# SebastianHafner/multimodal_siamese_cd

Hardware: AMD Instinct MI355X
Metric: image-pairs/sec training step, 256×256 SAR+optical Siamese U-Net, 1/2/4/8 MI355X (higher is better)
Workload: dtype f32 (h2 split-fp16); 1 GPU; baseline_siamese: siameseunet TOPOLOGY [64, 128, 256, 512], 5-ch SAR+optical, 256x256, bs=32/GPU, conv math h2, fp32 activation storage, train step incl. AdamW; global_batch=32, tile=256, parallelism=dp1

## Files before the change

### multimodal_siamese_cd_amd/csrc/bn_f32.hip

```cpp
#include "common.h"

namespace scd {

constexpr int BN_THREADS = 256;
constexpr int BN_CHUNK_MAX = 4096;
constexpr int BN_CHUNK_MIN = 64;
constexpr int BN_TARGET_BLOCKS = 2048;

struct BnGeom {
    int64_t pseg;
    int chunk;
    int ncps;
    int nrec;
    int qpb;
    int cgroups;
};

static BnGeom bn_geom(const scd_nhwc_t &y, int nseg) {
    BnGeom g;
    g.pseg = pixels(y) / nseg;
    const int cq = y.c / 4;
    int q = 1;
    while (q * 2 <= cq && q * 2 <= 64) q *= 2;
    g.qpb = q;
    g.cgroups = (cq + q - 1) / q;
    int chunk = BN_CHUNK_MAX;
    while (chunk > BN_CHUNK_MIN && int64_t(nseg) * ((g.pseg + chunk - 1) / chunk) * g.cgroups < BN_TARGET_BLOCKS)
        chunk /= 2;
    g.chunk = chunk;
    g.ncps = int((g.pseg + chunk - 1) / chunk);
    g.nrec = nseg * g.ncps;
    return g;
}

typedef float f4 __attribute__((ext_vector_type(4)));

__device__ __forceinline__ f4 fabs4(f4 v) { return f4{fabsf(v.x), fabsf(v.y), fabsf(v.z), fabsf(v.w)}; }
__device__ __forceinline__ f4 fmax4(f4 a, f4 b) {
    return f4{fmaxf(a.x, b.x), fmaxf(a.y, b.y), fmaxf(a.z, b.z), fmaxf(a.w, b.w)};
}
#define PIN4(a, b, c, d) asm volatile("" : "+v"(a), "+v"(b), "+v"(c), "+v"(d))

struct Welford4 {
    float n;
    f4 mean, m2;
};

__device__ __forceinline__ void chan_merge(Welford4 &a, const Welford4 &b) {
    if (b.n == 0.f) return;
    if (a.n == 0.f) {
        a = b;
        return;
// ... 80 lines not shown
        __syncthreads();
    }
    if (pl == 0 && c < C) {
        const Welford4 a = sh[tid];
        const float mv[4] = {a.mean.x, a.mean.y, a.mean.z, a.mean.w};
        const float qv[4] = {a.m2.x, a.m2.y, a.m2.z, a.m2.w};
#pragma unroll
        for (int k = 0; k < 4; ++k) {
            float *r = rec + (size_t(c + k) * nrec + blockIdx.x) * 3;
            r[0] = a.n;
            r[1] = mv[k];
            r[2] = qv[k];
        }
    }
}

struct DWelford {
    double n, mean, m2;
};
__device__ __forceinline__ void dmerge(DWelford &a, const DWelford &b) {
    if (b.n == 0) return;
    if (a.n == 0) {
        a = b;
        return;
    }
    const double n = a.n + b.n;
    const double d = b.mean - a.mean;
    a.mean += d * b.n / n;
    a.m2 += b.m2 + d * d * a.n * b.n / n;
    a.n = n;
}

__device__ __forceinline__ DWelford block_dmerge(DWelford w, DWelford *sh) {
#pragma unroll
    for (int off = 1; off < 64; off <<= 1) {
        const DWelford o{__shfl_xor(w.n, off), __shfl_xor(w.mean, off), __shfl_xor(w.m2, off)};
        dmerge(w, o);
    }
    const int t = threadIdx.x;
    if ((t & 63) == 0) sh[t >> 6] = w;
    __syncthreads();
    DWelford a = sh[0];
    if (t == 0)
        for (int k = 1; k < BN_THREADS / 64; ++k) dmerge(a, sh[k]);
    __syncthreads();
    return a;
}

__device__ __forceinline__ float bn_act_bound(double n, double gamma, double beta, double shift) {
    const double dev = fabs(gamma) * sqrt(n > 1 ? n - 1 : 0.0);
    return float((dev + fabs(beta)) * (1.0 + 0x1p-10) + (fabs(shift) + fabs(beta)) * 0x1p-16);
}

__global__ __launch_bounds__(BN_THREADS) void bn_stats_finalize(const float *__restrict__ rec, int C, int nseg,
                                                                int ncps, int nrec, const float *gamma,
                                                                const float *beta, float eps, float momentum,
                                                                int update, float *rmean, float *rvar, float *smean,
                                                                float *sinv, float *scale, float *shift,
                                                                float *act_bound) {
    __shared__ DWelford sh[BN_THREADS / 64];
    const int c = blockIdx.x;
    const int t = threadIdx.x;
    const float *rc = rec + size_t(c) * nrec * 3;
    for (int s = 0; s < nseg; ++s) {
        DWelford w{0, 0, 0};
        for (int k = t; k < ncps; k += BN_THREADS) {
            const float *r = rc + size_t(s * ncps + k) * 3;
            dmerge(w, DWelford{r[0], r[1], r[2]});
        }
        const DWelford a = block_dmerge(w, sh);
        if (t == 0) {
            const double g = gamma ? gamma[c] : 1.0, b = beta ? beta[c] : 0.0;
            const double var = a.n > 0 ? a.m2 / a.n : 0.0;
            const double inv = 1.0 / sqrt(var + double(eps));
            smean[s * C + c] = float(a.mean);
            sinv[s * C + c] = float(inv);
            const float sc = float(g * inv);
            scale[s * C + c] = sc;
            shift[s * C + c] = float(b - a.mean * double(sc));
            if (act_bound) atomic_max_bound(act_bound, bn_act_bound(a.n, g, b, double(shift[s * C + c])));
            if (update) {
                const double uvar = a.n > 1 ? a.m2 / (a.n - 1) : var;
                rmean[c] = float((1.0 - momentum) * rmean[c] + momentum * a.mean);
                rvar[c] = float((1.0 - momentum) * rvar[c] + momentum * uvar);
            }
        }
    }
}

__global__ __launch_bounds__(BN_THREADS) void bn_tile_merge(const float *__restrict__ trec, int C, int tiles_per_seg,
                                                            int group, int ncps, int nrec, float tile_px,
                                                            float *__restrict__ rec) {
    const int c = blockIdx.y * BN_THREADS + threadIdx.x;
    if (c >= C) return;
    const int g = blockIdx.x;
    const int seg = g / ncps, k = g - (g / ncps) * ncps;
    const int t0 = seg * tiles_per_seg + k * group;
    const int t1 = min(t0 + group, (seg + 1) * tiles_per_seg);
    float n = 0.f, mean = 0.f, m2 = 0.f;
    auto merge = [&](float2 r) {
        const float nn = n + tile_px;
        const float d = r.x - mean;
        mean += d * (tile_px / nn);
        m2 += r.y + d * d * (n * tile_px / nn);
        n = nn;
    };
    int t = t0;
    for (; t + 8 <= t1; t += 8) {
        float2 r[8];
#pragma unroll
        for (int u = 0; u < 8; ++u) r[u] = *reinterpret_cast<const float2 *>(trec + (size_t(t + u) * C + c) * 2);
#pragma unroll
        for (int u = 0; u < 8; ++u) merge(r[u]);
    }
    for (; t < t1; ++t) merge(*reinterpret_cast<const float2 *>(trec + (size_t(t) * C + c) * 2));
    float *o = rec + (size_t(c) * nrec + g) * 3;
    o[0] = n;
    o[1] = mean;
    o[2] = m2;
}

__global__ void bn_eval_coeffs_kernel(int C, const float *gamma, const float *beta, const float *rm, const float *rv,
                                      float eps, float *scale, float *shift) {
    const int c = blockIdx.x * blockDim.x + threadIdx.x;
    if (c >= C) return;
    const double inv = 1.0 / sqrt(double(rv[c]) + double(eps));
    const float sc = float((gamma ? gamma[c] : 1.0f) * inv);
    scale[c] = sc;
    shift[c] = float((beta ? beta[c] : 0.0f) - double(rm[c]) * sc);
}

__device__ __forceinline__ float bn_relu(float y, float sc, float sh) { return fmaxf(fmaf(y, sc, sh), 0.f); }
__device__ __forceinline__ f4 bn_relu4(f4 y, f4 sc, f4 sh) {
    return f4{bn_relu(y.x, sc.x, sh.x), bn_relu(y.y, sc.y, sh.y), bn_relu(y.z, sc.z, sh.z), bn_relu(y.w, sc.w, sh.w)};
}

template <class T>
__global__ __launch_bounds__(256) void bn_relu_apply_kernel(const T *__restrict__ y, int ldy, T *__restrict__ a,
                                                            int lda, int C, int64_t pseg, const float *__restrict__ scale,
                                                            const float *__restrict__ shift) {
    const int seg = blockIdx.y;
    const int cq = C / 4;
    const int64_t total = pseg * cq;
    const float *sc = scale + seg * C;
    const float *sh = shift + seg * C;
    for (int64_t e = blockIdx.x * int64_t(blockDim.x) + threadIdx.x; e < total; e += int64_t(gridDim.x) * blockDim.x) {
        const int64_t p = seg * pseg + e / cq;
        const int c = int(e % cq) * 4;
        st4(a + p * lda + c, bn_relu4(ld4(y + p * ldy + c), ld4(sc + c), ld4(sh + c)));
    }
}


template <class T>
struct DaPlain {
    const T *da;
    int ldda;
    __device__ __forceinline__ void bind(int) {}
    __device__ __forceinline__ f4 operator()(int64_t p, int c) const { return ld4(da + p * ldda + c); }
};
template <class T>
struct DaPooled {
    const T *gy;
    const uint8_t *idx;
    int hy, wy, ldgy;
    const T *gs;
    int gsn, ldgs, skip_mode;
    const T *gs2;
    int ldgs2;
    int hx, wx, C;
    FastDiv div_hw, div_w, div_gsn;
    __device__ __forceinline__ void bind(int) {}
// ... 566 lines not shown
#pragma unroll
            for (int k = 0; k < NO; ++k) hw[k] += (a0 * k0[k] + a1 * k1[k]) + (a2 * k2[k] + a3 * k3[k]);
        }
        for (; p < ch.end; p += npl) {
            const f4 y0 = ld4(y + p * ldy + c);
            f4 k0[NO];
            const f4 z0 = relu_mask(y0, sc, sf, px(p, y0, k0));
            s1 += z0;
            s2 += z0 * ((y0 - mu) * iv);
            const f4 a0 = bn_relu4(y0, sc, sf);
#pragma unroll
            for (int k = 0; k < NO; ++k) hw[k] += a0 * k0[k];
        }
    }
    sh1[tid] = s1;
    sh2[tid] = s2;
#pragma unroll
    for (int k = 0; k < NO; ++k) shh[k][tid] = hw[k];
    __syncthreads();
    for (int off = npl / 2; off > 0; off >>= 1) {
        if (pl < off) {
            sh1[tid] += sh1[tid + off * qpb];
            sh2[tid] += sh2[tid + off * qpb];
#pragma unroll
            for (int k = 0; k < NO; ++k) shh[k][tid] += shh[k][tid + off * qpb];
        }
        __syncthreads();
    }
    if (pl == 0 && c < C) {
        const f4 a = sh1[tid], b = sh2[tid];
        const float av[4] = {a.x, a.y, a.z, a.w}, bv[4] = {b.x, b.y, b.z, b.w};
#pragma unroll
        for (int k = 0; k < 4; ++k) {
            float *r = rec + (size_t(c + k) * nrec + blockIdx.x) * 2;
            r[0] = av[k];
            r[1] = bv[k];
        }
#pragma unroll
        for (int o = 0; o < NO; ++o) {
            const f4 h = shh[o][tid];
            const float hv[4] = {h.x, h.y, h.z, h.w};
#pragma unroll
            for (int k = 0; k < 4; ++k) hrec[(size_t(o) * C + c + k) * nrec + blockIdx.x] = hv[k];
        }
    }
}

__device__ __forceinline__ float bn_dy_bound(double da_bound, double n, double gamma, double mean, double inv, double k1,
                                             double k2) {
    const double xhat = sqrt(n > 1 ? n - 1 : 0.0) * (1.0 + 0x1p-10) + fabs(mean) * inv * 0x1p-20 + 1.0;
    return float(fabs(gamma * inv) * (da_bound + fabs(k1) + xhat * fabs(k2)) * (1.0 + 0x1p-10));
}

__global__ __launch_bounds__(BN_THREADS) void bn_bwd_finalize(const float *__restrict__ rec, int C, int nseg,
                                                              int ncps, int nrec, int64_t pseg, float *coef,
                                                              float *dgamma, float *dbeta, const float *gamma = nullptr,
                                                              const float *sinv = nullptr, float *dbias = nullptr,
                                                              const float *smean = nullptr,
                                                              const float *da_bound = nullptr,
                                                              float *dy_bound = nullptr) {
    __shared__ double a1[BN_THREADS], a2[BN_THREADS];
    const int c = blockIdx.x;
    const int t = threadIdx.x;
    const float *rc = rec + size_t(c) * nrec * 2;
    double tg = 0, tb = 0, db = 0;
    for (int s = 0; s < nseg; ++s) {
        double s1[4] = {0, 0, 0, 0}, s2[4] = {0, 0, 0, 0};
        const float2 *rs = reinterpret_cast<const float2 *>(rc) + size_t(s) * ncps;
        int k = t;
        for (; k + 3 * BN_THREADS < ncps; k += 4 * BN_THREADS) {
            float2 v[4];
#pragma unroll
            for (int u = 0; u < 4; ++u) v[u] = rs[k + u * BN_THREADS];
#pragma unroll
            for (int u = 0; u < 4; ++u) {
                s1[u] += v[u].x;
                s2[u] += v[u].y;
            }
        }
        for (int u = 0; k < ncps; k += BN_THREADS, ++u) {
            const float2 v = rs[k];
            s1[u] += v.x;
            s2[u] += v.y;
        }
        double v1 = (s1[0] + s1[1]) + (s1[2] + s1[3]), v2 = (s2[0] + s2[1]) + (s2[2] + s2[3]);
#pragma unroll
        for (int off = 1; off < 64; off <<= 1) {
            v1 += __shfl_xor(v1, off);
            v2 += __shfl_xor(v2, off);
        }
        if ((t & 63) == 0) {
            a1[t >> 6] = v1;
            a2[t >> 6] = v2;
        }
        __syncthreads();
        if (t == 0) {
            for (int k = 1; k < BN_THREADS / 64; ++k) {
                a1[0] += a1[k];
                a2[0] += a2[k];
            }
            const float k1 = float(a1[0] / double(pseg));
            const float k2 = float(a2[0] / double(pseg));
            coef[(s * C + c) * 2 + 0] = k1;
            coef[(s * C + c) * 2 + 1] = k2;
            if (dy_bound) atomic_max_bound(dy_bound, bn_dy_bound(double(*da_bound), double(pseg), gamma ? gamma[c] : 1.0,
                                                                 smean[s * C + c], sinv[s * C + c], k1, k2));
            tb += a1[0];
            tg += a2[0];
            if (dbias) {
                const float mul = (gamma ? gamma[c] : 1.f) * sinv[s * C + c];
                db += double(mul) * (a1[0] - double(pseg) * double(k1));
            }
        }
        __syncthreads();
    }
    if (t == 0) {
        if (dgamma) dgamma[c] = float(tg);
        if (dbeta) dbeta[c] = float(tb);
        if (dbias) dbias[c] = float(db);
    }
}

template <class T, class DA>
__global__ __launch_bounds__(BN_THREADS) void bn_bwd_apply(const T *__restrict__ y, int ldy, DA da,
                                                           T *__restrict__ dy, int lddy, int C, int64_t pseg,
                                                           int ncps, int chunk, int nrec, int qpb, const float *smean,
                                                           const float *sinv, const float *gamma, const float *scale,
                                                           const float *shift, const float *coef,
                                                           float *__restrict__ brec, float *dy_bound) {
    __shared__ f4 sh[BN_THREADS];
    const int tid = threadIdx.x;
    const int q = tid % qpb, pl = tid / qpb, npl = BN_THREADS / qpb;
    const int c = (blockIdx.y * qpb + q) * 4;
    const Chunk ch = chunk_of(pseg, ncps, chunk);
    f4 acc = {0.f, 0.f, 0.f, 0.f};
    f4 amax = acc;
    da.bind(c);
    if (c < C) {
        const int o = ch.seg * C + c;
        const f4 mu = ld4(smean + o), iv = ld4(sinv + o), sc = ld4(scale + o), sf = ld4(shift + o);
        const float *cf = coef + size_t(o) * 2;
        const f4 k1 = {cf[0], cf[2], cf[4], cf[6]};
        const f4 k2 = {cf[1], cf[3], cf[5], cf[7]};
        const f4 gm = gamma ? ld4(gamma + c) : f4{1.f, 1.f, 1.f, 1.f};
        const f4 mul = gm * iv;
        int64_t p = ch.beg + pl;
        for (; p + 3 * npl < ch.end; p += 4 * npl) {
            f4 y0 = ld4(y + p * ldy + c), y1 = ld4(y + (p + npl) * ldy + c);
            f4 y2 = ld4(y + (p + 2 * npl) * ldy + c), y3 = ld4(y + (p + 3 * npl) * ldy + c);
            f4 g0 = da(p, c), g1 = da(p + npl, c);
            f4 g2 = da(p + 2 * npl, c), g3 = da(p + 3 * npl, c);
            PIN4(y0, y1, y2, y3);
            PIN4(g0, g1, g2, g3);
            const f4 o0 = stored4(dy, bn_bwd_dy4(y0, g0, mu, iv, sc, sf, k1, k2, mul));
            const f4 o1 = stored4(dy, bn_bwd_dy4(y1, g1, mu, iv, sc, sf, k1, k2, mul));
            const f4 o2 = stored4(dy, bn_bwd_dy4(y2, g2, mu, iv, sc, sf, k1, k2, mul));
            const f4 o3 = stored4(dy, bn_bwd_dy4(y3, g3, mu, iv, sc, sf, k1, k2, mul));
            st4(dy + p * lddy + c, o0);
            st4(dy + (p + npl) * lddy + c, o1);
            st4(dy + (p + 2 * npl) * lddy + c, o2);
            st4(dy + (p + 3 * npl) * lddy + c, o3);
            acc += (o0 + o1) + (o2 + o3);
            if (dy_bound) amax = fmax4(amax, fmax4(fmax4(fabs4(o0), fabs4(o1)), fmax4(fabs4(o2), fabs4(o3))));
        }
        for (; p < ch.end; p += npl) {
            const f4 y0 = ld4(y + p * ldy + c);
            const f4 o0 = stored4(dy, bn_bwd_dy4(y0, da(p, c), mu, iv, sc, sf, k1, k2, mul));
            st4(dy + p * lddy + c, o0);
            acc += o0;
            if (dy_bound) amax = fmax4(amax, fabs4(o0));
        }
    }
    if (dy_bound) wave_max_bound(dy_bound, fmaxf(fmaxf(amax.x, amax.y), fmaxf(amax.z, amax.w)));
    if (!brec) return;
    sh[tid] = acc;
    __syncthreads();
    for (int off = npl / 2; off > 0; off >>= 1) {
        if (pl < off) sh[tid] += sh[tid + off * qpb];
        __syncthreads();
    }
    if (pl == 0 && c < C) {
        const f4 a = sh[tid];
        const float av[4] = {a.x, a.y, a.z, a.w};
#pragma unroll
        for (int k = 0; k < 4; ++k) brec[size_t(c + k) * nrec + blockIdx.x] = av[k];
    }
}

__global__ __launch_bounds__(BN_THREADS) void sum_records(const float *__restrict__ rec, int nrec, float *out) {
    __shared__ double sh[BN_THREADS];
    const int c = blockIdx.x;
    const int t = threadIdx.x;
    double s = 0;
    for (int k = t; k < nrec; k += BN_THREADS) s += rec[size_t(c) * nrec + k];
    sh[t] = s;
    __syncthreads();
    for (int off = BN_THREADS / 2; off > 0; off >>= 1) {
        if (t < off) sh[t] += sh[t + off];
        __syncthreads();
    }
    if (t == 0) out[c] = float(sh[0]);
}

template <class T>
__global__ __launch_bounds__(BN_THREADS) void chan_sum_partial(const T *__restrict__ x, int ldx, int C,
                                                               int64_t npix, int chunk, int nrec, int qpb,
                                                               const float *__restrict__ wgt, int hw, int n_out,
                                                               int o, const float *__restrict__ scale,
                                                               const float *__restrict__ shift, int64_t pseg,
                                                               float *__restrict__ rec) {
    __shared__ f4 sh[BN_THREADS];
    const int tid = threadIdx.x;
    const int q = tid % qpb, pl = tid / qpb, npl = BN_THREADS / qpb;
    const int c = (blockIdx.y * qpb + q) * 4;
    const int64_t pbeg = int64_t(blockIdx.x) * chunk;
    const int64_t pend = min(pbeg + chunk, npix);
    f4 acc = {0.f, 0.f, 0.f, 0.f};
    const bool small = npix < (int64_t(1) << 31);
    auto img_of = [&](int64_t p) { return small ? int64_t(uint32_t(p) / uint32_t(hw)) : p / hw; };
    auto seg_of = [&](int64_t p) { return small ? int64_t(uint32_t(p) / uint32_t(pseg)) : p / pseg; };
    auto wgt_at = [&](int64_t p) {
        const int64_t img = img_of(p), pix = p - img * hw;
        return wgt[(img * n_out + o) * hw + pix];
    };
    auto value = [&](int64_t p, f4 v, float wv) {
        if (scale) {
            const int64_t sc_off = seg_of(p) * C + c;
            v = bn_relu4(v, ld4(scale + sc_off), ld4(shift + sc_off));
        }
        if (wgt) v *= wv;
        return v;
    };
    if (c < C) {
        int64_t p = pbeg + pl;
        for (; p + 3 * npl < pend; p += 4 * npl) {
            f4 v0 = ld4(x + p * ldx + c), v1 = ld4(x + (p + npl) * ldx + c);
            f4 v2 = ld4(x + (p + 2 * npl) * ldx + c), v3 = ld4(x + (p + 3 * npl) * ldx + c);
            float w0 = 1.f, w1 = 1.f, w2 = 1.f, w3 = 1.f;
            if (wgt) {
                w0 = wgt_at(p);
                w1 = wgt_at(p + npl);
                w2 = wgt_at(p + 2 * npl);
                w3 = wgt_at(p + 3 * npl);
            }
            PIN4(v0, v1, v2, v3);
            if (wgt || scale) {
                v0 = value(p, v0, w0);
                v1 = value(p + npl, v1, w1);
                v2 = value(p + 2 * npl, v2, w2);
                v3 = value(p + 3 * npl, v3, w3);
            }
            acc += (v0 + v1) + (v2 + v3);
        }
        for (; p < pend; p += npl) acc += value(p, ld4(x + p * ldx + c), wgt ? wgt_at(p) : 1.f);
// ... 45 lines not shown
    SCD_WITH_T(x.dtype, T,
               hipLaunchKernelGGL(chan_sum_partial<T>, dim3(g.nrec, g.cgroups), dim3(BN_THREADS), 0, s,
                                  view_ptr<const T>(x), x.ldc, x.c, pixels(x), g.chunk, g.nrec, g.qpb, wgt, x.h * x.w,
                                  n_out, o, scale, shift, pixels(x) / nseg, rec));
    hipLaunchKernelGGL(sum_records, dim3(x.c), dim3(BN_THREADS), 0, s, rec, g.nrec, out);
    return SCD_OK;
}

}

using namespace scd;

extern "C" size_t scd_bn_workspace_bytes(int32_t n, int32_t h, int32_t w, int32_t c, int32_t nseg) {
    if (nseg < 1) nseg = 1;
    scd_nhwc_t v{nullptr, n, h, w, c, c};
    const BnGeom g = bn_geom(v, nseg);
    const size_t a = size_t(g.nrec) * c * 3;
    const size_t b = size_t(g.nrec) * c * 3 + size_t(nseg) * c * 2;
    return (a > b ? a : b) * sizeof(float) + 256;
}

extern "C" int scd_bn_train_stats(scd_nhwc_t y, int32_t nseg, const float *gamma, const float *beta, float eps,
                                  float momentum, int32_t update_running, float *running_mean, float *running_var,
                                  float *save_mean, float *save_invstd, float *scale, float *shift, float *act_bound,
                                  void *ws, size_t ws_bytes, scd_stream_t stream) {
    clear_error();
    SCD_TRY(bn_check(y, nseg));
    if (!save_mean || !save_invstd || !scale || !shift || (update_running && (!running_mean || !running_var))) {
        set_error("bn_train_stats: null output");
        return SCD_ERR_ARG;
    }
    if (!ws || ws_bytes < scd_bn_workspace_bytes(y.n, y.h, y.w, y.c, nseg)) {
        set_error("bn_train_stats: workspace too small");
        return SCD_ERR_WORKSPACE;
    }
    const BnGeom g = bn_geom(y, nseg);
    hipStream_t s = as_stream(stream);
    float *rec = static_cast<float *>(ws);
    SCD_WITH_T(y.dtype, T,
               hipLaunchKernelGGL(bn_stats_partial<T>, dim3(g.nrec, g.cgroups), dim3(BN_THREADS), 0, s,
                                  view_ptr<const T>(y), y.ldc, y.c, g.pseg, g.ncps, g.chunk, g.nrec, g.qpb, rec));
    hipLaunchKernelGGL(bn_stats_finalize, dim3(y.c), dim3(BN_THREADS), 0, s, rec, y.c, nseg, g.ncps, g.nrec, gamma,
                       beta, eps, momentum, update_running, running_mean, running_var, save_mean, save_invstd, scale,
                       shift, act_bound);
    return launch_status("scd_bn_train_stats");
}

static void tile_groups(int ntiles, int nseg, int *tiles_per_seg, int *group, int *ncps) {
    *tiles_per_seg = ntiles / nseg;
    *group = *tiles_per_seg / 256 > 1 ? *tiles_per_seg / 256 : 1;
    *ncps = (*tiles_per_seg + *group - 1) / *group;
}

extern "C" size_t scd_bn_tile_stats_workspace_bytes(int32_t ntiles, int32_t c, int32_t nseg) {
    if (nseg < 1 || ntiles < 1 || c < 1) return 0;
    int tps, group, ncps;
    tile_groups(ntiles, nseg, &tps, &group, &ncps);
    return size_t(nseg) * ncps * c * 3 * sizeof(float) + 256;
}

extern "C" int scd_bn_stats_from_tiles(const float *tile_rec, int32_t ntiles, int32_t tile_pixels, int32_t c,
                                       int32_t nseg, const float *gamma, const float *beta, float eps, float momentum,
                                       int32_t update_running, float *running_mean, float *running_var,
                                       float *save_mean, float *save_invstd, float *scale, float *shift,
                                       float *act_bound, void *ws, size_t ws_bytes, scd_stream_t stream) {
    clear_error();
    if (!tile_rec || ntiles < 1 || tile_pixels < 1 || c < 1 || nseg < 1 || ntiles % nseg || !save_mean ||
        !save_invstd || !scale || !shift || (update_running && (!running_mean || !running_var))) {
        set_error("bn_stats_from_tiles: bad arguments");
        return SCD_ERR_ARG;
    }
    if (!ws || ws_bytes < scd_bn_tile_stats_workspace_bytes(ntiles, c, nseg)) {
        set_error("bn_stats_from_tiles: workspace too small");
        return SCD_ERR_WORKSPACE;
    }
    int tps, group, ncps;
    tile_groups(ntiles, nseg, &tps, &group, &ncps);
    const int nrec = nseg * ncps;
    float *rec = static_cast<float *>(ws);
    hipStream_t s = as_stream(stream);
    hipLaunchKernelGGL(bn_tile_merge, dim3(nrec, (c + BN_THREADS - 1) / BN_THREADS), dim3(BN_THREADS), 0, s, tile_rec,
                       c, tps, group, ncps, nrec, float(tile_pixels), rec);
    hipLaunchKernelGGL(bn_stats_finalize, dim3(c), dim3(BN_THREADS), 0, s, rec, c, nseg, ncps, nrec, gamma, beta, eps,
                       momentum, update_running, running_mean, running_var, save_mean, save_invstd, scale, shift,
                       act_bound);
    return launch_status("scd_bn_stats_from_tiles");
}

extern "C" int scd_bn_eval_coeffs(int32_t c, const float *gamma, const float *beta, const float *running_mean,
                                  const float *running_var, float eps, float *scale, float *shift,
                                  scd_stream_t stream) {
    clear_error();
    if (c < 1 || !running_mean || !running_var || !scale || !shift) {
        set_error("bn_eval_coeffs: bad arguments");
        return SCD_ERR_ARG;
    }
    hipLaunchKernelGGL(bn_eval_coeffs_kernel, dim3((c + 127) / 128), dim3(128), 0, as_stream(stream), c, gamma, beta,
                       running_mean, running_var, eps, scale, shift);
    return launch_status("scd_bn_eval_coeffs");
}

extern "C" int scd_bn_relu_apply(scd_nhwc_t y, int32_t nseg, const float *scale, const float *shift, scd_nhwc_t a,
                                 scd_stream_t stream) {
    clear_error();
    SCD_TRY(bn_check(y, nseg));
    SCD_TRY(check_view(a, "bn_relu_apply.a"));
    if (a.n != y.n || a.h != y.h || a.w != y.w || a.c != y.c || !scale || !shift) {
        set_error("bn_relu_apply: shape mismatch");
        return SCD_ERR_ARG;
    }
    const int dt = common_dtype("bn_relu_apply", {&y, &a});
    if (dt < 0) return SCD_ERR_ARG;
    const int64_t pseg = pixels(y) / nseg;
    const int64_t total = pseg * (y.c / 4);
    int blocks = int((total + 255) / 256);
    if (blocks > 2048) blocks = 2048;
    SCD_WITH_T(dt, T,
               hipLaunchKernelGGL(bn_relu_apply_kernel<T>, dim3(blocks, nseg), dim3(256), 0, as_stream(stream),
                                  view_ptr<const T>(y), y.ldc, view_ptr<T>(a), a.ldc, y.c, pseg, scale, shift));
    return launch_status("scd_bn_relu_apply");
}

namespace scd {
template <class T, class DA>
static void bn_backward_run(const scd_nhwc_t &y, DA da, int nseg, const float *save_mean, const float *save_invstd,
                            const float *gamma, const float *scale, const float *shift, float *dgamma, float *dbeta,
                            float *dbias_prev, const scd_nhwc_t &dy, float *dy_bound, void *ws, hipStream_t s) {
    const BnGeom g = bn_geom(y, nseg);
    float *rec = static_cast<float *>(ws);
    float *brec = rec + size_t(g.nrec) * y.c * 2;
    float *coef = brec + size_t(g.nrec) * y.c;
    hipLaunchKernelGGL((bn_bwd_partial<T, DA>), dim3(g.nrec, g.cgroups), dim3(BN_THREADS), 0, s,
                       view_ptr<const T>(y), y.ldc, da, y.c, g.pseg, g.ncps, g.chunk, g.nrec, g.qpb,
                       save_mean, save_invstd, scale, shift, rec);
    hipLaunchKernelGGL(bn_bwd_finalize, dim3(y.c), dim3(BN_THREADS), 0, s, rec, y.c, nseg, g.ncps, g.nrec, g.pseg,
                       coef, dgamma, dbeta);
    hipLaunchKernelGGL((bn_bwd_apply<T, DA>), dim3(g.nrec, g.cgroups), dim3(BN_THREADS), 0, s,
                       view_ptr<const T>(y), y.ldc, da, view_ptr<T>(dy), dy.ldc, y.c,
                       g.pseg, g.ncps, g.chunk, g.nrec, g.qpb, save_mean, save_invstd, gamma, scale, shift, coef,
                       dbias_prev ? brec : nullptr, dy_bound);
    if (dbias_prev) hipLaunchKernelGGL(sum_records, dim3(y.c), dim3(BN_THREADS), 0, s, brec, g.nrec, dbias_prev);
}
template <class T, int NO>
static void bn_backward_run_head(const scd_nhwc_t &y, const DaHead &da, int nseg, const float *save_mean,
                                 const float *save_invstd, const float *gamma, const float *scale, const float *shift,
                                 float *dgamma, float *dbeta, float *dbias_prev, const scd_nhwc_t &dy, float *dy_bound,
                                 float *w_grad, void *ws, hipStream_t s) {
    const BnGeom g = bn_geom(y, nseg);
    float *rec = static_cast<float *>(ws);
    float *brec = rec + size_t(g.nrec) * y.c * 2;
    float *coef = brec + size_t(g.nrec) * y.c;
    float *hrec = reinterpret_cast<float *>(static_cast<unsigned char *>(ws) +
                                            scd_bn_workspace_bytes(y.n, y.h, y.w, y.c, nseg));
    hipLaunchKernelGGL((bn_bwd_partial_head<T, NO>), dim3(g.nrec, g.cgroups), dim3(BN_THREADS), 0, s,
                       view_ptr<const T>(y), y.ldc, da, y.c, g.pseg, g.ncps, g.chunk, g.nrec, g.qpb,
                       save_mean, save_invstd, scale, shift, rec, hrec);
    hipLaunchKernelGGL(bn_bwd_finalize, dim3(y.c), dim3(BN_THREADS), 0, s, rec, y.c, nseg, g.ncps, g.nrec, g.pseg,
                       coef, dgamma, dbeta);
    hipLaunchKernelGGL((bn_bwd_apply<T, DaHeadN<NO>>), dim3(g.nrec, g.cgroups), dim3(BN_THREADS), 0, s,
                       view_ptr<const T>(y), y.ldc, DaHeadN<NO>{da, {}}, view_ptr<T>(dy), dy.ldc, y.c,
                       g.pseg, g.ncps, g.chunk, g.nrec, g.qpb, save_mean, save_invstd, gamma, scale, shift, coef,
                       dbias_prev ? brec : nullptr, dy_bound);
    if (dbias_prev) hipLaunchKernelGGL(sum_records, dim3(y.c), dim3(BN_THREADS), 0, s, brec, g.nrec, dbias_prev);
    hipLaunchKernelGGL(sum_records, dim3(da.n_out * y.c), dim3(BN_THREADS), 0, s, hrec, g.nrec, w_grad);
}
#ifndef SCD_BN_POOLED_CELLS
#define SCD_BN_POOLED_CELLS 1
#endif
#ifndef SCD_BN_POOLED_PAIR
#define SCD_BN_POOLED_PAIR 1
#endif
template <class T, bool S2>
static void bn_backward_pooled_cells(const scd_nhwc_t &y, const PooledCells<T> &P, int nseg, const BnGeom &g,
                                     int64_t cseg, int chunk, int ncps, int nrec, const float *save_mean,
                                     const float *save_invstd, const float *gamma, const float *scale,
                                     const float *shift, float *dgamma, float *dbeta, float *dbias_prev,
                                     const scd_nhwc_t &dy, float *dy_bound, float *rec, float *brec, float *coef,
                                     hipStream_t s);
template <class T>
static void bn_backward_run_pooled(const scd_nhwc_t &y, const DaPooled<T> &da, int nseg, const float *save_mean,
                                   const float *save_invstd, const float *gamma, const float *scale, const float *shift,
                                   float *dgamma, float *dbeta, float *dbias_prev, const scd_nhwc_t &dy,
                                   float *dy_bound, void *ws, hipStream_t s) {
    if (!SCD_BN_POOLED_CELLS) {
        bn_backward_run<T>(y, da, nseg, save_mean, save_invstd, gamma, scale, shift, dgamma, dbeta, dbias_prev, dy,
                           dy_bound, ws, s);
        return;
    }
    const BnGeom g = bn_geom(y, nseg);
    PooledCells<T> P;
    P.da = da;
    P.ch = (y.h + 1) / 2;
    P.cw = (y.w + 1) / 2;
    P.div_cimg = make_fastdiv(uint32_t(P.ch * P.cw));
    P.div_cw = make_fastdiv(uint32_t(P.cw));
    const int64_t cseg = int64_t(y.n / nseg) * P.ch * P.cw;
    const int chunk = int((cseg + g.ncps - 1) / g.ncps);
    const int ncps = int((cseg + chunk - 1) / chunk);
    const int nrec = nseg * ncps;
    float *rec = static_cast<float *>(ws);
    float *brec = rec + size_t(g.nrec) * y.c * 2;
    float *coef = brec + size_t(g.nrec) * y.c;
    if (da.gs2) {
        bn_backward_pooled_cells<T, true>(y, P, nseg, g, cseg, chunk, ncps, nrec, save_mean, save_invstd, gamma, scale,
                                          shift, dgamma, dbeta, dbias_prev, dy, dy_bound, rec, brec, coef, s);
    } else {
        bn_backward_pooled_cells<T, false>(y, P, nseg, g, cseg, chunk, ncps, nrec, save_mean, save_invstd, gamma, scale,
                                           shift, dgamma, dbeta, dbias_prev, dy, dy_bound, rec, brec, coef, s);
    }
}

template <class T, bool S2>
static void bn_backward_pooled_cells(const scd_nhwc_t &y, const PooledCells<T> &P, int nseg, const BnGeom &g,
                                     int64_t cseg, int chunk, int ncps, int nrec, const float *save_mean,
                                     const float *save_invstd, const float *gamma, const float *scale,
                                     const float *shift, float *dgamma, float *dbeta, float *dbias_prev,
                                     const scd_nhwc_t &dy, float *dy_bound, float *rec, float *brec, float *coef,
// ... 307 lines not shown
```

### multimodal_siamese_cd_amd/csrc/conv_f32.hip

```cpp
#include <algorithm>

#include "conv_common.h"

namespace scd {

template <int WAVES_M, int WAVES_N, int TM, int TN, int BK>
__global__ __launch_bounds__(64 * WAVES_M *WAVES_N) void igemm_f32(IgemmArgs a) {
    constexpr int NT = 64 * WAVES_M * WAVES_N;
    constexpr int BM = WAVES_M * TM * 32;
    constexpr int BN = WAVES_N * TN * 32;
    constexpr int LS = BK + 4;
    constexpr int KC = BK / 4;
    constexpr int A_CH = BM * KC;
    constexpr int B_CH = BN * KC;
    constexpr int A_PER = (A_CH + NT - 1) / NT;
    constexpr int B_PER = (B_CH + NT - 1) / NT;
    constexpr int STAGE = (BM + BN) * LS;
    __shared__ __attribute__((aligned(16))) float smem[2 * STAGE];

    const int tid = threadIdx.x;
    const int lane = tid & 63;
    const int wid = tid >> 6;
    const int wm = wid % WAVES_M;
    const int wn = wid / WAVES_M;
// ... 1208 lines not shown
    if (d->src_scale || d->src_shift) {
        if (!d->src_scale || !d->src_shift || d->src_nseg < 1 || d->src.n % d->src_nseg ||
            !aligned16(d->src_scale) || !aligned16(d->src_shift) || !wgrad_src_bn_ok(d)) {
            set_error("wgrad: src transform needs both 16-byte aligned coefficient arrays, src_nseg | src.n and a "
                      "supported shape (check scd_wgrad_src_bn_supported)");
            return SCD_ERR_ARG;
        }
        a.src_seg_imgs = d->src.n / d->src_nseg;
    }
    if (wgrad_halo_ok(d)) {
        a.n_img_w = d->rows.n;
        a.grid_r = a.R / wgrad_halo_rblock(a.math, a.tune, a.R, wgrad_bounded(d));
        a.grid_j = a.C / 64;
        a.remap = xcd_remap_enabled(a.tune);
        launch_wgrad_halo16_x3(a, dim3(a.grid_r * a.grid_j * ns), s);
        return launch_status("scd_conv_wgrad");
    }
    if (wgrad_c16_ok(d)) {
        a.n_img_w = d->rows.n;
        a.grid_r = a.R / 64;
        a.grid_j = 1;
        a.remap = xcd_remap_enabled(a.tune);
        launch_wgrad_halo16_c16(a, dim3(a.grid_r * ns), s);
        return launch_status("scd_conv_wgrad");
    }
    const WgradTile t = wgrad_tile(a.R, Ng);
    a.grid_r = (a.R + t.bm - 1) / t.bm;
    a.grid_j = (Ng + t.bn - 1) / t.bn;
    a.remap = xcd_remap_enabled(a.tune);
    dim3 grid(a.grid_r * a.grid_j * ns);
    dim3 block(t.threads);
    if (math_split(a.math)) {
        if (wgrad_generic_h2(d))
            launch_wgrad_x3_h2(a, t.id, grid, block, s);
        else if (wgrad_generic_bf16(d))
            launch_wgrad_x3_bf16(a, t.id, grid, block, s);
        else
            launch_wgrad_x3(a, t.id, grid, block, s);
        return launch_status("scd_conv_wgrad");
    }
    switch (t.id) {
        case 0: hipLaunchKernelGGL((wgrad_f32<2, 2, 2, 2, 16>), grid, block, 0, s, a); break;
        case 1: hipLaunchKernelGGL((wgrad_f32<1, 4, 2, 2, 16>), grid, block, 0, s, a); break;
        case 2: hipLaunchKernelGGL((wgrad_f32<2, 2, 1, 3, 16>), grid, block, 0, s, a); break;
        case 3: hipLaunchKernelGGL((wgrad_f32<2, 1, 1, 3, 16>), grid, block, 0, s, a); break;
        default: hipLaunchKernelGGL((wgrad_f32<1, 4, 1, 1, 16>), grid, block, 0, s, a); break;
    }
    return launch_status("scd_conv_wgrad");
}
}

namespace scd {
constexpr int kColsumGroup = 16;
__global__ __launch_bounds__(256) void colsum_group_kernel(float *__restrict__ colsum, int nsplit, int Ng) {
    const int j = blockIdx.x * 256 + threadIdx.x;
    if (j >= Ng) return;
    const int s0 = blockIdx.y * kColsumGroup, s1 = min(s0 + kColsumGroup, nsplit);
    float v[kColsumGroup];
#pragma unroll
    for (int u = 0; u < kColsumGroup; ++u) v[u] = s0 + u < s1 ? colsum[size_t(s0 + u) * Ng + j] : 0.f;
    float acc = 0.f;
#pragma unroll
    for (int u = 0; u < kColsumGroup; ++u) acc += v[u];
    colsum[size_t(s0) * Ng + j] = acc;
}
__global__ __launch_bounds__(256) void colsum_final_kernel(const float *__restrict__ colsum, int nsplit, int ntaps,
                                                           int C, float *__restrict__ out) {
    const int c = blockIdx.x * 256 + threadIdx.x;
    if (c >= C) return;
    const int Ng = ntaps * C;
    float tap[9];
#pragma unroll
    for (int t = 0; t < 9; ++t) tap[t] = 0.f;
#pragma unroll 4
    for (int s = 0; s < nsplit; s += kColsumGroup)
#pragma unroll
        for (int t = 0; t < 9; ++t)
            if (t < ntaps) tap[t] += colsum[size_t(s) * Ng + t * C + c];
    float acc = 0.f;
#pragma unroll
    for (int t = 0; t < 9; ++t)
        if (t < ntaps) acc += tap[t];
    out[c] = acc;
}
}

extern "C" int scd_wgrad_colsum_finalize(float *colsum, int32_t nsplit, int32_t ntaps, int32_t C, float *out,
                                         scd_stream_t stream) {
    clear_error();
    if (!colsum || !out || nsplit < 1 || ntaps < 1 || ntaps > 9 || C < 1) {
        set_error("wgrad_colsum_finalize: colsum/out non-null, nsplit=%d >= 1, ntaps=%d in [1, 9], C=%d >= 1", nsplit,
                  ntaps, C);
        return SCD_ERR_ARG;
    }
    const hipStream_t s = as_stream(stream);
    const int Ng = ntaps * C;
    hipLaunchKernelGGL(colsum_group_kernel, dim3((Ng + 255) / 256, (nsplit + kColsumGroup - 1) / kColsumGroup),
                       dim3(256), 0, s, colsum, nsplit, Ng);
    hipLaunchKernelGGL(colsum_final_kernel, dim3((C + 255) / 256), dim3(256), 0, s, colsum, nsplit, ntaps, C, out);
    return launch_status("scd_wgrad_colsum_finalize");
}

extern "C" int scd_wgrad_finalize(float *slabs, int32_t nsplit, int32_t R, int32_t ntaps, int32_t C,
                                  int32_t mode, int32_t c_valid, float *out, scd_stream_t stream) {
    clear_error();
    if (!slabs || !out || nsplit < 1 || R < 1 || ntaps < 1 || C < 1 || (mode != 0 && mode != 1) || c_valid < 1 ||
        c_valid > C) {
        set_error("wgrad_finalize: bad arguments");
        return SCD_ERR_ARG;
    }
    const size_t total = size_t(R) * ntaps * C;
    const int base_blocks = int((total + 255) / 256);
    hipStream_t s = as_stream(stream);
    int G = (2048 + base_blocks - 1) / base_blocks;
    if (G > (nsplit + 3) / 4) G = (nsplit + 3) / 4;
    if (G < 1) G = 1;
    int nsum = nsplit, gstride = 1;
    if (G > 1) {
        const int per = (nsplit + G - 1) / G;
        G = (nsplit + per - 1) / per;
        if (total % 4 == 0 && aligned16(slabs))
            hipLaunchKernelGGL(wgrad_group_sum4, dim3(unsigned((total / 4 + 255) / 256), G), dim3(256), 0, s, slabs,
                               nsplit, per, total);
        else
            hipLaunchKernelGGL(wgrad_group_sum, dim3(base_blocks, G), dim3(256), 0, s, slabs, nsplit, per, total);
        nsum = G;
        gstride = per;
    }
    if (ntaps <= kFinMaxTaps) {
        hipLaunchKernelGGL(wgrad_finalize_rows, dim3(R, (C + kFinCB - 1) / kFinCB), dim3(256), 0, s, slabs, nsum,
                           gstride, R, ntaps, C, mode, c_valid, out);
        return launch_status("scd_wgrad_finalize");
    }
    const int blocks = base_blocks > 4096 ? 4096 : base_blocks;
    hipLaunchKernelGGL(wgrad_finalize_kernel, dim3(blocks), dim3(256), 0, s, slabs, nsum, gstride, R, ntaps, C, mode,
                       c_valid, out);
    return launch_status("scd_wgrad_finalize");
}
```

Measured before the change: 1105 image-pairs/s.

## Fuse BN tile-merge with stats finalize, bwd finalize with head sum, colsum passes

```diff
diff --git a/multimodal_siamese_cd_amd/csrc/bn_f32.hip b/multimodal_siamese_cd_amd/csrc/bn_f32.hip
--- a/multimodal_siamese_cd_amd/csrc/bn_f32.hip
+++ b/multimodal_siamese_cd_amd/csrc/bn_f32.hip
@@ -1,3 +1,5 @@
+#include <cstdlib>
+
 #include "common.h"
 
 namespace scd {
@@ -184,6 +186,26 @@
     return float((dev + fabs(beta)) * (1.0 + 0x1p-10) + (fabs(shift) + fabs(beta)) * 0x1p-16);
 }
 
+__device__ __forceinline__ void bn_stats_emit(const DWelford &a, int s, int c, int C, const float *gamma,
+                                              const float *beta, float eps, float momentum, int update, float *rmean,
+                                              float *rvar, float *smean, float *sinv, float *scale, float *shift,
+                                              float *act_bound) {
+    const double g = gamma ? gamma[c] : 1.0, b = beta ? beta[c] : 0.0;
+    const double var = a.n > 0 ? a.m2 / a.n : 0.0;
+    const double inv = 1.0 / sqrt(var + double(eps));
+    smean[s * C + c] = float(a.mean);
+    sinv[s * C + c] = float(inv);
+    const float sc = float(g * inv);
+    scale[s * C + c] = sc;
+    shift[s * C + c] = float(b - a.mean * double(sc));
+    if (act_bound) atomic_max_bound(act_bound, bn_act_bound(a.n, g, b, double(shift[s * C + c])));
+    if (update) {
+        const double uvar = a.n > 1 ? a.m2 / (a.n - 1) : var;
+        rmean[c] = float((1.0 - momentum) * rmean[c] + momentum * a.mean);
+        rvar[c] = float((1.0 - momentum) * rvar[c] + momentum * uvar);
+    }
+}
+
 __global__ __launch_bounds__(BN_THREADS) void bn_stats_finalize(const float *__restrict__ rec, int C, int nseg,
                                                                 int ncps, int nrec, const float *gamma,
                                                                 const float *beta, float eps, float momentum,
@@ -201,34 +223,17 @@
             dmerge(w, DWelford{r[0], r[1], r[2]});
         }
         const DWelford a = block_dmerge(w, sh);
-        if (t == 0) {
-            const double g = gamma ? gamma[c] : 1.0, b = beta ? beta[c] : 0.0;
-            const double var = a.n > 0 ? a.m2 / a.n : 0.0;
-            const double inv = 1.0 / sqrt(var + double(eps));
-            smean[s * C + c] = float(a.mean);
-            sinv[s * C + c] = float(inv);
-            const float sc = float(g * inv);
-            scale[s * C + c] = sc;
-            shift[s * C + c] = float(b - a.mean * double(sc));
-            if (act_bound) atomic_max_bound(act_bound, bn_act_bound(a.n, g, b, double(shift[s * C + c])));
-            if (update) {
-                const double uvar = a.n > 1 ? a.m2 / (a.n - 1) : var;
-                rmean[c] = float((1.0 - momentum) * rmean[c] + momentum * a.mean);
-                rvar[c] = float((1.0 - momentum) * rvar[c] + momentum * uvar);
-            }
-        }
-    }
-}
-
-__global__ __launch_bounds__(BN_THREADS) void bn_tile_merge(const float *__restrict__ trec, int C, int tiles_per_seg,
-                                                            int group, int ncps, int nrec, float tile_px,
-                                                            float *__restrict__ rec) {
-    const int c = blockIdx.y * BN_THREADS + threadIdx.x;
-    if (c >= C) return;
-    const int g = blockIdx.x;
-    const int seg = g / ncps, k = g - (g / ncps) * ncps;
-    const int t0 = seg * tiles_per_seg + k * group;
-    const int t1 = min(t0 + group, (seg + 1) * tiles_per_seg);
+        if (t == 0)
+            bn_stats_emit(a, s, c, C, gamma, beta, eps, momentum, update, rmean, rvar, smean, sinv, scale, shift,
+                          act_bound);
+    }
+}
+
+struct TileChunk {
+    float n, mean, m2;
+};
+__device__ __forceinline__ TileChunk tile_chunk(const float *__restrict__ trec, int C, int c, int t0, int t1,
+                                                float tile_px) {
     float n = 0.f, mean = 0.f, m2 = 0.f;
     auto merge = [&](float2 r) {
         const float nn = n + tile_px;
@@ -246,10 +251,68 @@
         for (int u = 0; u < 8; ++u) merge(r[u]);
     }
     for (; t < t1; ++t) merge(*reinterpret_cast<const float2 *>(trec + (size_t(t) * C + c) * 2));
+    return TileChunk{n, mean, m2};
+}
+
+__global__ __launch_bounds__(BN_THREADS) void bn_tile_merge(const float *__restrict__ trec, int C, int tiles_per_seg,
+                                                            int group, int ncps, int nrec, float tile_px,
+                                                            float *__restrict__ rec) {
+    const int c = blockIdx.y * BN_THREADS + threadIdx.x;
+    if (c >= C) return;
+    const int g = blockIdx.x;
+    const int seg = g / ncps, k = g - (g / ncps) * ncps;
+    const int t0 = seg * tiles_per_seg + k * group;
+    const int t1 = min(t0 + group, (seg + 1) * tiles_per_seg);
+    const TileChunk r = tile_chunk(trec, C, c, t0, t1, tile_px);
     float *o = rec + (size_t(c) * nrec + g) * 3;
-    o[0] = n;
-    o[1] = mean;
-    o[2] = m2;
+    o[0] = r.n;
+    o[1] = r.mean;
+    o[2] = r.m2;
+}
+
+constexpr int kTileFusedGroupMax = 7;
+__device__ __forceinline__ TileChunk tile_chunk_short(const float *__restrict__ trec, int C, int c, int t0, int t1,
+                                                      float tile_px) {
+#pragma clang fp contract(off)
+    float2 r[kTileFusedGroupMax];
+#pragma unroll
+    for (int u = 0; u < kTileFusedGroupMax; ++u)
+        r[u] = t0 + u < t1 ? *reinterpret_cast<const float2 *>(trec + (size_t(t0 + u) * C + c) * 2) : float2{0.f, 0.f};
+    float n = 0.f, mean = 0.f, m2 = 0.f;
+#pragma unroll
+    for (int u = 0; u < kTileFusedGroupMax; ++u) {
+        if (t0 + u < t1) {
+            const float nn = n + tile_px;
+            const float d = r[u].x - mean;
+            mean = __builtin_fmaf(d, tile_px / nn, mean);
+            m2 = m2 + __builtin_fmaf(d * d, n * tile_px / nn, r[u].y);
+            n = nn;
+        }
+    }
+    return TileChunk{n, mean, m2};
+}
+__global__ __launch_bounds__(BN_THREADS) void bn_tile_stats_fused(const float *__restrict__ trec, int C, int nseg,
+                                                                  int tiles_per_seg, int group, int ncps,
+                                                                  float tile_px, const float *gamma, const float *beta,
+                                                                  float eps, float momentum, int update, float *rmean,
+                                                                  float *rvar, float *smean, float *sinv, float *scale,
+                                                                  float *shift, float *act_bound) {
+    __shared__ DWelford sh[BN_THREADS / 64];
+    const int c = blockIdx.x;
+    const int t = threadIdx.x;
+    for (int s = 0; s < nseg; ++s) {
+        DWelford w{0, 0, 0};
+        for (int k = t; k < ncps; k += BN_THREADS) {
+            const int t0 = s * tiles_per_seg + k * group;
+            const int t1 = min(t0 + group, (s + 1) * tiles_per_seg);
+            const TileChunk r = tile_chunk_short(trec, C, c, t0, t1, tile_px);
+            dmerge(w, DWelford{r.n, r.mean, r.m2});
+        }
+        const DWelford a = block_dmerge(w, sh);
+        if (t == 0)
+            bn_stats_emit(a, s, c, C, gamma, beta, eps, momentum, update, rmean, rvar, smean, sinv, scale, shift,
+                          act_bound);
+    }
 }
 
 __global__ void bn_eval_coeffs_kernel(int C, const float *gamma, const float *beta, const float *rm, const float *rv,
@@ -922,15 +985,11 @@
     return float(fabs(gamma * inv) * (da_bound + fabs(k1) + xhat * fabs(k2)) * (1.0 + 0x1p-10));
 }
 
-__global__ __launch_bounds__(BN_THREADS) void bn_bwd_finalize(const float *__restrict__ rec, int C, int nseg,
-                                                              int ncps, int nrec, int64_t pseg, float *coef,
-                                                              float *dgamma, float *dbeta, const float *gamma = nullptr,
-                                                              const float *sinv = nullptr, float *dbias = nullptr,
-                                                              const float *smean = nullptr,
-                                                              const float *da_bound = nullptr,
-                                                              float *dy_bound = nullptr) {
-    __shared__ double a1[BN_THREADS], a2[BN_THREADS];
-    const int c = blockIdx.x;
+__device__ __forceinline__ void bn_bwd_finalize_channel(int c, double *a1, double *a2, const float *__restrict__ rec,
+                                                        int C, int nseg, int ncps, int nrec, int64_t pseg, float *coef,
+                                                        float *dgamma, float *dbeta, const float *gamma,
+                                                        const float *sinv, float *dbias, const float *smean,
+                                                        const float *da_bound, float *dy_bound) {
     const int t = threadIdx.x;
     const float *rc = rec + size_t(c) * nrec * 2;
     double tg = 0, tb = 0, db = 0;
@@ -989,6 +1048,17 @@
         if (dbeta) dbeta[c] = float(tb);
         if (dbias) dbias[c] = float(db);
     }
+}
+__global__ __launch_bounds__(BN_THREADS) void bn_bwd_finalize(const float *__restrict__ rec, int C, int nseg,
+                                                              int ncps, int nrec, int64_t pseg, float *coef,
+                                                              float *dgamma, float *dbeta, const float *gamma = nullptr,
+                                                              const float *sinv = nullptr, float *dbias = nullptr,
+                                                              const float *smean = nullptr,
+                                                              const float *da_bound = nullptr,
+                                                              float *dy_bound = nullptr) {
+    __shared__ double a1[BN_THREADS / 64], a2[BN_THREADS / 64];
+    bn_bwd_finalize_channel(blockIdx.x, a1, a2, rec, C, nseg, ncps, nrec, pseg, coef, dgamma, dbeta, gamma, sinv, dbias,
+                            smean, da_bound, dy_bound);
 }
 
 template <class T, class DA>
@@ -1057,9 +1127,8 @@
     }
 }
 
-__global__ __launch_bounds__(BN_THREADS) void sum_records(const float *__restrict__ rec, int nrec, float *out) {
-    __shared__ double sh[BN_THREADS];
-    const int c = blockIdx.x;
+__device__ __forceinline__ void sum_records_channel(int c, double *sh, const float *__restrict__ rec, int nrec,
+                                                    float *out) {
     const int t = threadIdx.x;
     double s = 0;
     for (int k = t; k < nrec; k += BN_THREADS) s += rec[size_t(c) * nrec + k];
@@ -1070,6 +1139,23 @@
         __syncthreads();
     }
     if (t == 0) out[c] = float(sh[0]);
+}
+__global__ __launch_bounds__(BN_THREADS) void sum_records(const float *__restrict__ rec, int nrec, float *out) {
+    __shared__ double sh[BN_THREADS];
+    sum_records_channel(blockIdx.x, sh, rec, nrec, out);
+}
+__global__ __launch_bounds__(BN_THREADS) void bn_bwd_finalize_and_sum(const float *__restrict__ rec, int C, int nseg,
+                                                                      int ncps, int nrec, int64_t pseg, float *coef,
+                                                                      float *dgamma, float *dbeta,
+                                                                      const float *__restrict__ srec, int snrec,
+                                                                      float *sout) {
+    __shared__ double sh[BN_THREADS];
+    if (int(blockIdx.x) < C) {
+        bn_bwd_finalize_channel(blockIdx.x, sh, sh + BN_THREADS / 64, rec, C, nseg, ncps, nrec, pseg, coef, dgamma,
+                                dbeta, nullptr, nullptr, nullptr, nullptr, nullptr, nullptr);
+    } else {
+        sum_records_channel(blockIdx.x - C, sh, srec, snrec, sout);
+    }
 }
 
 template <class T>
@@ -1221,6 +1307,12 @@
     *ncps = (*tiles_per_seg + *group - 1) / *group;
 }
 
+constexpr int BN_TILE_FUSED_MAX = 1024;
+static int tile_fused_max() {
+    const char *e = getenv("SCD_BN_TILE_FUSED_MAX");
+    return e && *e ? atoi(e) : BN_TILE_FUSED_MAX;
+}
+
 extern "C" size_t scd_bn_tile_stats_workspace_bytes(int32_t ntiles, int32_t c, int32_t nseg) {
     if (nseg < 1 || ntiles < 1 || c < 1) return 0;
     int tps, group, ncps;
@@ -1248,6 +1340,12 @@
     const int nrec = nseg * ncps;
     float *rec = static_cast<float *>(ws);
     hipStream_t s = as_stream(stream);
+    if (tps <= tile_fused_max() && group <= kTileFusedGroupMax) {
+        hipLaunchKernelGGL(bn_tile_stats_fused, dim3(c), dim3(BN_THREADS), 0, s, tile_rec, c, nseg, tps, group, ncps,
+                           float(tile_pixels), gamma, beta, eps, momentum, update_running, running_mean, running_var,
+                           save_mean, save_invstd, scale, shift, act_bound);
+        return launch_status("scd_bn_stats_from_tiles");
+    }
     hipLaunchKernelGGL(bn_tile_merge, dim3(nrec, (c + BN_THREADS - 1) / BN_THREADS), dim3(BN_THREADS), 0, s, tile_rec,
                        c, tps, group, ncps, nrec, float(tile_pixels), rec);
     hipLaunchKernelGGL(bn_stats_finalize, dim3(c), dim3(BN_THREADS), 0, s, rec, c, nseg, ncps, nrec, gamma, beta, eps,
@@ -1324,14 +1422,13 @@
     hipLaunchKernelGGL((bn_bwd_partial_head<T, NO>), dim3(g.nrec, g.cgroups), dim3(BN_THREADS), 0, s,
                        view_ptr<const T>(y), y.ldc, da, y.c, g.pseg, g.ncps, g.chunk, g.nrec, g.qpb,
                        save_mean, save_invstd, scale, shift, rec, hrec);
-    hipLaunchKernelGGL(bn_bwd_finalize, dim3(y.c), dim3(BN_THREADS), 0, s, rec, y.c, nseg, g.ncps, g.nrec, g.pseg,
-                       coef, dgamma, dbeta);
+    hipLaunchKernelGGL(bn_bwd_finalize_and_sum, dim3(y.c + da.n_out * y.c), dim3(BN_THREADS), 0, s, rec, y.c, nseg,
+                       g.ncps, g.nrec, g.pseg, coef, dgamma, dbeta, hrec, g.nrec, w_grad);
     hipLaunchKernelGGL((bn_bwd_apply<T, DaHeadN<NO>>), dim3(g.nrec, g.cgroups), dim3(BN_THREADS), 0, s,
                        view_ptr<const T>(y), y.ldc, DaHeadN<NO>{da, {}}, view_ptr<T>(dy), dy.ldc, y.c,
                        g.pseg, g.ncps, g.chunk, g.nrec, g.qpb, save_mean, save_invstd, gamma, scale, shift, coef,
                        dbias_prev ? brec : nullptr, dy_bound);
     if (dbias_prev) hipLaunchKernelGGL(sum_records, dim3(y.c), dim3(BN_THREADS), 0, s, brec, g.nrec, dbias_prev);
-    hipLaunchKernelGGL(sum_records, dim3(da.n_out * y.c), dim3(BN_THREADS), 0, s, hrec, g.nrec, w_grad);
 }
 #ifndef SCD_BN_POOLED_CELLS
 #define SCD_BN_POOLED_CELLS 1
diff --git a/multimodal_siamese_cd_amd/csrc/conv_f32.hip b/multimodal_siamese_cd_amd/csrc/conv_f32.hip
--- a/multimodal_siamese_cd_amd/csrc/conv_f32.hip
+++ b/multimodal_siamese_cd_amd/csrc/conv_f32.hip
@@ -1284,36 +1284,46 @@
 
 namespace scd {
 constexpr int kColsumGroup = 16;
-__global__ __launch_bounds__(256) void colsum_group_kernel(float *__restrict__ colsum, int nsplit, int Ng) {
-    const int j = blockIdx.x * 256 + threadIdx.x;
-    if (j >= Ng) return;
-    const int s0 = blockIdx.y * kColsumGroup, s1 = min(s0 + kColsumGroup, nsplit);
-    float v[kColsumGroup];
-#pragma unroll
-    for (int u = 0; u < kColsumGroup; ++u) v[u] = s0 + u < s1 ? colsum[size_t(s0 + u) * Ng + j] : 0.f;
-    float acc = 0.f;
-#pragma unroll
-    for (int u = 0; u < kColsumGroup; ++u) acc += v[u];
-    colsum[size_t(s0) * Ng + j] = acc;
-}
-__global__ __launch_bounds__(256) void colsum_final_kernel(const float *__restrict__ colsum, int nsplit, int ntaps,
-                                                           int C, float *__restrict__ out) {
-    const int c = blockIdx.x * 256 + threadIdx.x;
-    if (c >= C) return;
+constexpr int kColsumChan = 4;
+__global__ __launch_bounds__(256) void colsum_finalize_kernel(const float *__restrict__ colsum, int nsplit, int ntaps,
+                                                              int C, float *__restrict__ out) {
+    __shared__ float grp[256];
+    __shared__ float taps[9 * kColsumChan];
+    const int i = threadIdx.x;
+    const int per = ntaps * kColsumChan;
+    const int gp = 256 / per;
+    const int cl = i % kColsumChan, t = (i / kColsumChan) % ntaps, gl = i / per;
+    const int c = blockIdx.x * kColsumChan + cl;
     const int Ng = ntaps * C;
-    float tap[9];
-#pragma unroll
-    for (int t = 0; t < 9; ++t) tap[t] = 0.f;
-#pragma unroll 4
-    for (int s = 0; s < nsplit; s += kColsumGroup)
-#pragma unroll
-        for (int t = 0; t < 9; ++t)
-            if (t < ntaps) tap[t] += colsum[size_t(s) * Ng + t * C + c];
-    float acc = 0.f;
-#pragma unroll
-    for (int t = 0; t < 9; ++t)
-        if (t < ntaps) acc += tap[t];
-    out[c] = acc;
+    const int ngroups = (nsplit + kColsumGroup - 1) / kColsumGroup;
+    float tap = 0.f;
+    for (int g0 = 0; g0 < ngroups; g0 += gp) {
+        const int g = g0 + gl;
+        if (gl < gp && g < ngroups && c < C) {
+            const int s0 = g * kColsumGroup, s1 = min(s0 + kColsumGroup, nsplit);
+            const int j = t * C + c;
+            float v[kColsumGroup];
+#pragma unroll
+            for (int u = 0; u < kColsumGroup; ++u) v[u] = s0 + u < s1 ? colsum[size_t(s0 + u) * Ng + j] : 0.f;
+            float acc = 0.f;
+#pragma unroll
+            for (int u = 0; u < kColsumGroup; ++u) acc += v[u];
+            grp[i] = acc;
+        }
+        __syncthreads();
+        if (i < per && c < C) {
+            const int n = min(gp, ngroups - g0);
+            for (int k = 0; k < n; ++k) tap += grp[k * per + i];
+        }
+        __syncthreads();
+    }
+    if (i < per) taps[i] = tap;
+    __syncthreads();
+    if (i < kColsumChan && c < C) {
+        float acc = 0.f;
+        for (int k = 0; k < ntaps; ++k) acc += taps[k * kColsumChan + i];
+        out[c] = acc;
+    }
 }
 }
 
@@ -1326,10 +1336,8 @@
         return SCD_ERR_ARG;
     }
     const hipStream_t s = as_stream(stream);
-    const int Ng = ntaps * C;
-    hipLaunchKernelGGL(colsum_group_kernel, dim3((Ng + 255) / 256, (nsplit + kColsumGroup - 1) / kColsumGroup),
-                       dim3(256), 0, s, colsum, nsplit, Ng);
-    hipLaunchKernelGGL(colsum_final_kernel, dim3((C + 255) / 256), dim3(256), 0, s, colsum, nsplit, ntaps, C, out);
+    hipLaunchKernelGGL(colsum_finalize_kernel, dim3((C + kColsumChan - 1) / kColsumChan), dim3(256), 0, s, colsum, nsplit,
+                       ntaps, C, out);
     return launch_status("scd_wgrad_colsum_finalize");
 }
 
```

Result: no change. 1104 image-pairs/s (-0.0%).
